# p2004dr/visual-slam

Measured on AMD Instinct MI355X. Metric: frames/sec (extract+match+pose) at 640×480, 2000 ORB, 1/2/4/8 MI355X, higher is better.
Workload: dtype u8

## Files before the change

### visual-slam_amd/csrc/orb_kernels.hip

```cpp
#include <type_traits>
#include <cstring>

#include "common.h"
#include "select_replay.h"
#include "fast_score.h"

__constant__ __attribute__((aligned(16))) int8_t c_pattern[256 * 4] = {
#include "orb_pattern.inc"
};

#define WAVE 64

__device__ __forceinline__ int reflect101(int p, int len) {
    if (len == 1) return 0;
    while (p < 0 || p >= len) p = p < 0 ? -p : 2 * len - 2 - p;
    return p;
}

__device__ __forceinline__ void xcd_map(uint32_t lin, uint32_t per, uint32_t inv_per, uint32_t batch, int& frame, int& item) {
    const uint32_t b8 = batch & ~7u, cut = per * b8;
    const bool head = lin < cut;
    const uint32_t n = head ? lin >> 3 : lin - cut;
    const uint32_t q = inv_per ? __umulhi(n, inv_per) : n;
    item = (int)(n - q * per);
// ... 915 lines not shown
                                              int* flags, replay::WgScratch<NT>* ws, uint32_t (*s_hw)[27] , int level) {
    const int tid = threadIdx.x;
    constexpr int HG_GROUPS = NT / HG;
    if ((lv.pitch & 3) == 0 && (((size_t)img) & 3) == 0) {
        const int grp = tid / HG, g = tid % HG;
#ifndef SEL_HB
#define SEL_HB 4
#endif
        constexpr int HB = SEL_HB;
        for (int i0 = 0; i0 < N1; i0 += HG_GROUPS * HB) {
            uint32_t e[HB], reg[HB][4];
#pragma unroll
            for (int u = 0; u < HB; u++) {
                e[u] = A[min(i0 + u * HG_GROUPS + grp, N1 - 1)];
                harris_fetch(img, lv.pitch, e[u] & 0xFFF, (e[u] >> 12) & 0xFFF, g, reg[u]);
            }
#pragma unroll
            for (int u = 0; u < HB; u++) {
                const int i = i0 + u * HG_GROUPS + grp;
                const float r = harris_group(reg[u], e[u] & 0xFFF, s_hw[grp], g);
                if (g == 0 && i < N1) B[i] = ((uint64_t)__float_as_uint(r) << 32) | (e[u] & 0xFFFFFFu);
            }
        }
    } else {
        for (int i = tid; i < N1; i += NT) {
            uint32_t e = A[i];
            int x = e & 0xFFF, y = (e >> 12) & 0xFFF;
            float r = harris_response(img, lv.pitch, x, y);
            B[i] = ((uint64_t)__float_as_uint(r) << 32) | (e & 0xFFFFFFu);
        }
    }
    __syncthreads();
    int N2 = replay::wg_retain_best<NT, uint64_t>(B, N1, lv.quota, P.select_order, rpos, bl, tid, ws);
    if (N2 > lv.fin_cap) {
        if (tid == 0) { atomicOr(&flags[0], 1); atomicOr(&flags[1], 1 << level); }
        N2 = lv.fin_cap;
    }
    for (int i = tid; i < N2; i += NT) {
        uint64_t e = B[i];
        FinalKp k;
        k.x = (uint16_t)(e & 0xFFF);
        k.y = (uint16_t)((e >> 12) & 0xFFF);
        k.response = __uint_as_float((uint32_t)(e >> 32));
        fin[i] = k;
    }
    if (tid == 0) *fin_cnt_out = N2;
}

template <int NT>
__global__ __launch_bounds__(NT) void k_select(Plan P, const uint8_t* __restrict__ gray, const uint8_t* __restrict__ pyr,
                                                        const uint32_t* __restrict__ cand, const int* __restrict__ strip_cnt,
                                                        uint64_t* __restrict__ scratch, size_t scratch_stride,
                                                        FinalKp* __restrict__ fin_all, int* __restrict__ fin_cnt, int* flags,
                                                        int level0, int buf_bytes, int* __restrict__ desc_todo) {
    extern __shared__ __attribute__((aligned(16))) uint8_t s_buf[];
    int* const s_pref = (int*)(s_buf + buf_bytes);
    __shared__ replay::WgScratch<NT> s_ws;
    __shared__ uint32_t s_hw[NT / HG][27];
    const int L = level0 + blockIdx.y, frame = blockIdx.x, tid = threadIdx.x;
    if (desc_todo && frame == 0 && blockIdx.y == 0 && tid == 0) desc_todo[0] = 0;
    const LevelInfo lv = P.lv[L];
    int* fin_cnt_out = &fin_cnt[(size_t)frame * MO_MAX_LEVELS + L];
    if (lv.nstrips == 0) {
        if (tid == 0) *fin_cnt_out = 0;
        return;
    }
    const int* cnts = strip_cnt + (size_t)frame * P.strips_per_frame + lv.strip_base;
    for (int s = tid; s < lv.nstrips; s += NT) s_pref[s + 1] = cnts[s];
    __syncthreads();
    if (tid == 0) {
        s_pref[0] = 0;
        for (int s = 0; s < lv.nstrips; s++) s_pref[s + 1] += s_pref[s];
    }
    __syncthreads();
    const int N = s_pref[lv.nstrips];
    uint64_t* scr = scratch + (size_t)frame * scratch_stride + lv.scr_off;
    uint64_t* gB = scr;
    uint32_t* gA = (uint32_t*)(scr + lv.cand_cap);
    uint16_t* g_rpos = (uint16_t*)(gA + lv.cand_cap + (lv.cand_cap & 1));
    unsigned long long* g_bl = (unsigned long long*)(g_rpos + (((size_t)lv.cand_cap / 2 + 4) & ~(size_t)3));
    const bool a_lds = sel_need_bytes(N, 4) <= (size_t)buf_bytes;
    uint32_t* s_A = (uint32_t*)s_buf;
    uint16_t* a_rpos = (uint16_t*)(s_buf + (((size_t)N * 4 + 7) & ~(size_t)7));
    unsigned long long* a_bl = (unsigned long long*)((uint8_t*)a_rpos + ((((size_t)N / 2 + 1) * 2 + 7) & ~(size_t)7));
    const uint32_t* src = cand + (size_t)frame * P.cand_stride + lv.cand_off;
    {
        const int lane = tid & 63, wv = tid >> 6;
        constexpr int NW = NT / 64, GU = 4;
        for (int s0 = wv; s0 < lv.nstrips; s0 += NW * GU) {
            uint32_t v[GU];
            int b[GU], n[GU];
#pragma unroll
            for (int u = 0; u < GU; u++) {
                const int st = min(s0 + u * NW, lv.nstrips - 1);
                b[u] = s_pref[st];
                n[u] = s0 + u * NW < lv.nstrips ? s_pref[st + 1] - b[u] : 0;
                v[u] = lane < n[u] ? src[(size_t)st * lv.strip_cap + lane] : 0u;
            }
#pragma unroll
            for (int u = 0; u < GU; u++) {
                if (lane < n[u]) { if (a_lds) s_A[b[u] + lane] = v[u]; else gA[b[u] + lane] = v[u]; }
                if (n[u] > WAVE) {
                    const uint32_t* e = src + (size_t)(s0 + u * NW) * lv.strip_cap;
                    for (int i = WAVE + lane; i < n[u]; i += WAVE) { if (a_lds) s_A[b[u] + i] = e[i]; else gA[b[u] + i] = e[i]; }
                }
            }
        }
    }
    __syncthreads();
    const int N1 = a_lds ? replay::wg_retain_best<NT, uint32_t>(s_A, N, 2 * lv.quota, P.select_order, a_rpos, a_bl, tid, &s_ws)
                         : replay::wg_retain_best<NT, uint32_t>(gA, N, 2 * lv.quota, P.select_order, g_rpos, g_bl, tid, &s_ws);
    const size_t b_off = a_lds ? (((size_t)N1 * 4 + 15) & ~(size_t)15) : 0;
    const bool b_lds = b_off + sel_need_bytes(N1, 8) <= (size_t)buf_bytes;
    uint64_t* s_B = (uint64_t*)(s_buf + b_off);
    uint16_t* b_rpos = (uint16_t*)((uint8_t*)s_B + (size_t)N1 * 8);
    unsigned long long* b_bl = (unsigned long long*)((uint8_t*)b_rpos + ((((size_t)N1 / 2 + 1) * 2 + 7) & ~(size_t)7));
    const uint8_t* img = level_ptr(P, L, gray, pyr, frame);
    FinalKp* fin = fin_all + (size_t)frame * P.fin_stride + lv.fin_off;
    if (a_lds && b_lds) select_harris<NT>(P, lv, img, s_A, s_B, N1, b_rpos, b_bl, fin, fin_cnt_out, flags, &s_ws, s_hw, L);
    else if (a_lds) select_harris<NT>(P, lv, img, s_A, gB, N1, g_rpos, g_bl, fin, fin_cnt_out, flags, &s_ws, s_hw, L);
    else if (b_lds) select_harris<NT>(P, lv, img, gA, s_B, N1, b_rpos, b_bl, fin, fin_cnt_out, flags, &s_ws, s_hw, L);
    else select_harris<NT>(P, lv, img, gA, gB, N1, g_rpos, g_bl, fin, fin_cnt_out, flags, &s_ws, s_hw, L);
}

int orb_launch_select(mo_ctx* c, const uint8_t* d_gray, int batch, int level_lo, int level_hi) {
    const Plan& P = c->plan;
    level_lo = std::max(level_lo, 0); level_hi = std::min(level_hi, P.nlevels);
    if (level_lo >= level_hi) return MO_OK;
    const size_t pref_bytes = (((size_t)c->pb.max_strips + 1) * sizeof(int) + 15) & ~(size_t)15;
    const size_t attr_bytes = SEL_BUF_BYTES + ((((size_t)SEL_MAXSTRIPS + 1) * sizeof(int) + 15) & ~(size_t)15);
    int rc;
    if ((rc = mo_raise_dyn_lds(c, (const void*)k_select<SEL_THREADS>, (int)attr_bytes)) ||
        (rc = mo_raise_dyn_lds(c, (const void*)k_select<SEL_THREADS_LATENCY>, (int)attr_bytes)))
        return rc;
    const dim3 grid(batch, level_hi - level_lo);
    if (batch <= 2)
        hipLaunchKernelGGL(k_select<SEL_THREADS_LATENCY>, grid, dim3(SEL_THREADS_LATENCY), SEL_BUF_BYTES + pref_bytes, c->stream, P, d_gray, c->pb.d_pyr, c->pb.d_cand,
                           c->pb.d_strip_cnt, c->pb.d_scratch, c->pb.scratch_stride, c->pb.d_fin, c->pb.d_fin_cnt, c->flags_cur, level_lo, SEL_BUF_BYTES, c->pb.d_dtodo);
    else
        hipLaunchKernelGGL(k_select<SEL_THREADS>, grid, dim3(SEL_THREADS), SEL_BUF_BYTES + pref_bytes, c->stream, P, d_gray, c->pb.d_pyr, c->pb.d_cand,
                           c->pb.d_strip_cnt, c->pb.d_scratch, c->pb.scratch_stride, c->pb.d_fin, c->pb.d_fin_cnt, c->flags_cur, level_lo, SEL_BUF_BYTES, c->pb.d_dtodo);
    HIPCHK(c, hipGetLastError());
    return MO_OK;
}

__global__ __launch_bounds__(SEL_THREADS) void k_retain_probe(const float* resp, int n, int n_points, int order, uint64_t* rec,
                                                              uint16_t* rpos, unsigned long long* bl, int32_t* out, int* nout) {
    __shared__ replay::WgScratch<SEL_THREADS> s_ws;
    for (int i = threadIdx.x; i < n; i += SEL_THREADS) rec[i] = ((uint64_t)__float_as_uint(resp[i]) << 32) | (uint32_t)i;
    __syncthreads();
    int keep = replay::wg_retain_best<SEL_THREADS, uint64_t>(rec, n, n_points, order, rpos, bl, threadIdx.x, &s_ws);
    __syncthreads();
    for (int i = threadIdx.x; i < keep; i += SEL_THREADS) out[i] = (int32_t)(rec[i] & 0xFFFFFFFFu);
    if (threadIdx.x == 0) *nout = keep;
}

int orb_launch_retain_probe(mo_ctx* c, const float* d_resp, int n, int n_points, int order, int32_t* d_order, int* d_nout) {
    size_t nn = (size_t)std::max(n, 1);
    size_t rec_b = nn * sizeof(uint64_t), rpos_b = ((nn / 2 + 4) * 2 + 7) & ~(size_t)7, bl_b = (nn / 64 + 8) * 8;
    int rc = c->d_tmp.reserve_exact(c, rec_b + rpos_b + bl_b);
    if (rc) return rc;
    uint8_t* b = c->d_tmp;
    hipLaunchKernelGGL(k_retain_probe, dim3(1), dim3(SEL_THREADS), 0, c->stream, d_resp, n, n_points, order, (uint64_t*)b,
                       (uint16_t*)(b + rec_b), (unsigned long long*)(b + rec_b + rpos_b), d_order, d_nout);
    HIPCHK(c, hipGetLastError());
    return MO_OK;
}

__device__ __forceinline__ float fast_atan2_deg(float y, float x) {
    const float p1 = 0.9997878412794807f * (float)(180 / 3.14159265358979323846);
    const float p3 = -0.3258083974640975f * (float)(180 / 3.14159265358979323846);
    const float p5 = 0.1555786518463281f * (float)(180 / 3.14159265358979323846);
    const float p7 = -0.04432655554792128f * (float)(180 / 3.14159265358979323846);
    float ax = fabsf(x), ay = fabsf(y);
    float a, c, c2;
    if (ax >= ay) {
        c = ay / (ax + (float)2.2204460492503131e-16);
        c2 = c * c;
        a = (((p7 * c2 + p5) * c2 + p3) * c2 + p1) * c;
    } else {
        c = ax / (ay + (float)2.2204460492503131e-16);
        c2 = c * c;
        a = 90.f - (((p7 * c2 + p5) * c2 + p3) * c2 + p1) * c;
    }
    if (x < 0) a = 180.f - a;
    if (y < 0) a = 360.f - a;
    return a;
}

__device__ __forceinline__ int wave_sum(int v) {
#pragma unroll
    for (int o = 32; o > 0; o >>= 1) v += __shfl_xor(v, o, 64);
    return v;
}

template <bool BOUNDS>
__device__ __forceinline__ void rbrief_wave(const uint8_t* blur, int bpitch, const uint8_t* raw, int rpitch, int lw, int lh,
                                            int cx, int cy, float angle_deg, uint8_t* desc, int lane) {
    float angle = angle_deg;
    angle *= (float)(3.14159265358979323846 / 180.f);
    double sd, cd;
    sincos((double)angle, &sd, &cd);
    float a = (float)cd, b = (float)sd;
    unsigned nib = 0;
#pragma unroll
    for (int k = 0; k < 4; k++) {
        const int8_t* pt = &c_pattern[(lane * 4 + k) * 4];
        float fx0 = (float)pt[0], fy0 = (float)pt[1], fx1 = (float)pt[2], fy1 = (float)pt[3];
        int ix0 = __float2int_rn(fx0 * a - fy0 * b), iy0 = __float2int_rn(fx0 * b + fy0 * a);
        int ix1 = __float2int_rn(fx1 * a - fy1 * b), iy1 = __float2int_rn(fx1 * b + fy1 * a);
        int x0 = cx + ix0, y0 = cy + iy0, x1 = cx + ix1, y1 = cy + iy1;
        int t0, t1;
        if (BOUNDS) {
            t0 = (x0 >= 0 && x0 < lw && y0 >= 0 && y0 < lh) ? blur[(size_t)y0 * bpitch + x0]
                                                           : raw[(size_t)reflect101(y0, lh) * rpitch + reflect101(x0, lw)];
            t1 = (x1 >= 0 && x1 < lw && y1 >= 0 && y1 < lh) ? blur[(size_t)y1 * bpitch + x1]
                                                           : raw[(size_t)reflect101(y1, lh) * rpitch + reflect101(x1, lw)];
        } else {
            t0 = blur[(size_t)y0 * bpitch + x0];
            t1 = blur[(size_t)y1 * bpitch + x1];
        }
        nib |= (t0 < t1 ? 1u : 0u) << k;
    }
    unsigned hi = __shfl_down(nib, 1, 64);
    if ((lane & 1) == 0) desc[lane >> 1] = (uint8_t)(nib | (hi << 4));
}

#define DG 16

__device__ __forceinline__ int group_sum(int v) {
#pragma unroll
    for (int o = DG / 2; o > 0; o >>= 1) v += __shfl_xor(v, o, 64);
    return v;
}

typedef const __attribute__((address_space(3))) uint8_t lds_cu8;
__device__ __forceinline__ uint16_t rbrief_u16_lds(uint32_t lds_base, int ppitch, float a, float b, const float4* pat, int gl) {
    const uint32_t base = lds_base - 0x4B400000u - 0x400000u * (uint32_t)ppitch;
    uint32_t val = 0;
#ifndef RB_UNROLL
#define RB_UNROLL 16
#endif
#pragma unroll 1
    for (int k0 = 16 - RB_UNROLL; k0 >= 0; k0 -= RB_UNROLL) {
#pragma unroll
        for (int kk = RB_UNROLL - 1; kk >= 0; kk--) {
            const float4 pt = pat[(k0 + kk) * DG + gl];
            const int jx0 = __float_as_int((pt.x * a - pt.y * b) + 12582912.f), jy0 = __float_as_int((pt.x * b + pt.y * a) + 12582912.f);
            const int jx1 = __float_as_int((pt.z * a - pt.w * b) + 12582912.f), jy1 = __float_as_int((pt.z * b + pt.w * a) + 12582912.f);
            const uint32_t a0 = (uint32_t)__mul24(jy0, ppitch) + (base + (uint32_t)jx0), a1 = (uint32_t)__mul24(jy1, ppitch) + (base + (uint32_t)jx1);
            const int t0 = *(lds_cu8*)(uintptr_t)a0, t1 = *(lds_cu8*)(uintptr_t)a1;
            val = __builtin_amdgcn_alignbit(val, (uint32_t)(t0 - t1), 31);
        }
    }
    return (uint16_t)val;
}

#define DT_RAW_P ((DT_W + 30 + 15 + 15) & ~15)
#define DT_RAW_ROWS (DT_H + 30)
#define DT_BLR_P ((DT_W + 38 + 15 + 15) & ~15)
#define DT_BLR_ROWS (DT_H + 38)
#define DT_RAW_NQ ((DT_W + 30 + 7 + 7) >> 3)
#define DT_BLR_NQ ((DT_W + 38 + 7 + 7) >> 3)
static_assert(((DT_RAW_P / 4) & 1) || ((DT_RAW_P / 4) & 7) == 4, "raw tile pitch: odd, or an odd multiple of 4 dwords");
#ifndef DT_NT
#define DT_NT 256
#endif
#ifdef DT_WAVES
#define DT_WAVES_ATTR __attribute__((amdgpu_waves_per_eu(DT_WAVES, 8)))
#else
#define DT_WAVES_ATTR
#endif
#define DT_CHUNK 512
#define DT_LIST (DT_NT > 160 ? DT_NT : 160)
#define DT_RAW_LD ((DT_RAW_ROWS * DT_RAW_NQ + DT_NT - 1) / DT_NT)
#define DT_BLR_LD ((DT_BLR_ROWS * DT_BLR_NQ + DT_NT - 1) / DT_NT)
#define DT_RAW_NP (DT_RAW_P / 16)
#define DT_BLR_NP (DT_BLR_P / 16)
#define DT_RAW_LD16 ((DT_RAW_ROWS + DT_NT / DT_RAW_NP - 1) / (DT_NT / DT_RAW_NP))
#define DT_BLR_LD16 ((DT_BLR_ROWS + DT_NT / DT_BLR_NP - 1) / (DT_NT / DT_BLR_NP))
#define DT_MAX2(a, b) ((a) > (b) ? (a) : (b))
#define DT_STAGE_REGS DT_MAX2(DT_MAX2(2 * DT_RAW_LD, 2 * DT_BLR_LD), DT_MAX2(4 * DT_RAW_LD16, 4 * DT_BLR_LD16))

template <int NROWS, int NQ, int NLD>
__device__ __forceinline__ void tile_issue(const uint8_t* img, int pitch, int h, int ry0, int cx_al, int tid, uint32_t (&v)[DT_STAGE_REGS]) {
    const int last_q = (pitch >> 3) - 1;
#pragma unroll
    for (int u = 0; u < NLD; u++) {
        const int t = min(tid + u * DT_NT, NROWS * NQ - 1), r = t / NQ, c = t - r * NQ;
        const int y = min(max(ry0 + r, 0), h - 1), q = min(max((cx_al >> 3) + c, 0), last_q);
        const uint2 d = ((const uint2*)(img + (size_t)y * pitch))[q];
        v[2 * u] = d.x; v[2 * u + 1] = d.y;
    }
}
template <int NROWS, int NQ, int LP, int NLD>
__device__ __forceinline__ void tile_store(uint8_t* lds, int tid, const uint32_t (&v)[DT_STAGE_REGS]) {
#pragma unroll
    for (int u = 0; u < NLD; u++) {
        const int t = tid + u * DT_NT, r = t / NQ, c = t - r * NQ;
        if (t < NROWS * NQ) *(uint2*)(lds + r * LP + 8 * c) = make_uint2(v[2 * u], v[2 * u + 1]);
    }
}
typedef uint32_t dt_u32x4 __attribute__((ext_vector_type(4)));
template <int NP>
__device__ __forceinline__ void tile_lane16(int pitch, int ry0, int cx_al, int nrows, int ncols, int tid, uint32_t& goff, uint32_t& loff, int& rows_left,
                                            uint32_t& last) {
    const int g = tid / NP, l = tid - g * NP;
    const bool on = g < DT_NT / NP && 16 * l < ncols && g < nrows;
    rows_left = on ? nrows - g : 0;
    goff = (uint32_t)(ry0 * pitch + cx_al) + (on ? (uint32_t)(g * pitch + 16 * l) : 0u);
    loff = (uint32_t)(g * (NP * 16) + 16 * l);
    last = on ? (uint32_t)((rows_left - 1) / (DT_NT / NP) * (DT_NT / NP) * pitch) : 0u;
}
template <int NP, int NLD>
__device__ __forceinline__ void tile_issue16(const uint8_t* img, int pitch, uint32_t goff, uint32_t last, uint32_t (&v)[DT_STAGE_REGS]) {
#pragma unroll
    for (int u = 0; u < NLD; u++) {
        const dt_u32x4 d = *(const dt_u32x4*)(img + (goff + min((uint32_t)(u * (DT_NT / NP) * pitch), last)));
        v[4 * u] = d.x; v[4 * u + 1] = d.y; v[4 * u + 2] = d.z; v[4 * u + 3] = d.w;
    }
}
template <int NP, int NLD>
__device__ __forceinline__ void tile_store16(uint8_t* lds, uint32_t loff, int rows_left, const uint32_t (&v)[DT_STAGE_REGS]) {
#pragma unroll
    for (int u = 0; u < NLD; u++)
        if (u * (DT_NT / NP) < rows_left) *(dt_u32x4*)(lds + loff + u * (DT_NT / NP) * (NP * 16)) = dt_u32x4{v[4 * u], v[4 * u + 1], v[4 * u + 2], v[4 * u + 3]};
}
__device__ __forceinline__ void tile_load_bytes(const uint8_t* img, int pitch, int w, int h, int ry0, int nrows, int cx0, int lp, uint8_t* lds, int tid) {
    for (int i = tid; i < nrows * lp; i += DT_NT) {
        const int r = i / lp, c = i - r * lp;
        const int y = min(max(ry0 + r, 0), h - 1), x = min(max(cx0 + c, 0), w - 1);
        lds[i] = img[(size_t)y * pitch + x];
    }
}

template <bool HAS_DESC, bool RARE>
__device__ __forceinline__ void describe_tile(const Plan& P, int frame, int tile, int tiles_per_frame, int split, int nsplit ,
                                              const uint32_t* __restrict__ tile_tab,
                                              const uint8_t* __restrict__ gray, const uint8_t* __restrict__ pyr,
                                              const uint8_t* __restrict__ blur, const FinalKp* __restrict__ fin_all,
                                              const int* __restrict__ fin_cnt, mo_keypoint* __restrict__ kps,
                                              uint8_t* __restrict__ desc, int cap, int* __restrict__ counts, int* flags,
                                              const uint32_t* __restrict__ icw, int* __restrict__ todo) {
    __shared__ __attribute__((aligned(16))) uint8_t s_tile[HAS_DESC ? DT_BLR_ROWS * DT_BLR_P : DT_RAW_ROWS * DT_RAW_P];
    __shared__ __attribute__((aligned(16))) float4 s_pat[HAS_DESC ? 256 : 1];
    __shared__ uint32_t s_list[DT_LIST];
    __shared__ float2 s_ab[DT_LIST];
    __shared__ int s_n;
    static_assert(DT_BLR_ROWS * DT_BLR_P >= DT_RAW_ROWS * DT_RAW_P, "the blurred tile is the larger one");
    const uint32_t te = tile_tab[tile];
    const int L = te & 0xFF;
    const int x0 = P.lv[L].bx0 + (int)((te >> 8) & 0xFFF) * DT_W, y0 = P.lv[L].by0 + (int)(te >> 20) * DT_H;
    const int lpitch = P.lv[L].pitch, lbpitch = P.lv[L].bpitch, lw = P.lv[L].w, lh = P.lv[L].h;
    const float lscale = P.lv[L].scale;
    const int tid = threadIdx.x, grp = tid / DG, gl = tid % DG;
    const int* fc = fin_cnt + (size_t)frame * MO_MAX_LEVELS;
    int total = 0, base = 0, nL = 0;
    {
        int cn[MO_MAX_LEVELS];
#pragma unroll
        for (int l = 0; l < MO_MAX_LEVELS; l++) cn[l] = fc[l];
#pragma unroll
        for (int l = 0; l < MO_MAX_LEVELS; l++) {
            const int n = l < P.nlevels ? cn[l] : 0;
            if (l == L) { base = total; nL = n; }
            total += n;
        }
    }
    if (!RARE && tile == 0 && split == 0 && tid == 0) {
        counts[frame] = total;
        if (total > cap) atomicOr(&flags[0], 2);
    }
    nL = min(nL, max(cap - base, 0));
    if (nL == 0) return;
    const uint8_t* img = level_ptr(P, L, gray, pyr, frame);
    const uint8_t* bl = blur + (size_t)frame * P.blur_stride + P.lv[L].boff;
    const bool al_raw = (lpitch & 7) == 0 && (((size_t)img) & 7) == 0;
    const bool al_blr = (((size_t)bl) & 7) == 0;
    const int nkc = min(DT_W, P.lv[L].bx0 + P.lv[L].bw - x0), nkr = min(DT_H, P.lv[L].by0 + P.lv[L].bh - y0);
    const int lead_r16 = (x0 - 15) & 15, lead_b16 = (x0 - 19) & 15;
    const int ncols_r = lead_r16 + nkc + 30, ncols_b = lead_b16 + nkc + 38;
    const bool w16_raw = !RARE && ((lpitch | (int)(size_t)img) & 15) == 0 && y0 - 15 >= 0 && y0 + nkr + 15 <= lh && x0 - 15 - lead_r16 >= 0 &&
                         x0 - 15 - lead_r16 + ((ncols_r + 15) & ~15) <= lpitch;
    const bool w16_blr = !RARE && ((lbpitch | (int)(size_t)bl) & 15) == 0 && y0 - 19 >= 0 && y0 + nkr + 19 <= lh && x0 - 19 - lead_b16 >= 0 &&
                         x0 - 19 - lead_b16 + ((ncols_b + 15) & ~15) <= lbpitch;
    const int xr_al = w16_raw ? x0 - 15 - lead_r16 : al_raw ? (x0 - 15) & ~7 : x0 - 15, lead_r = (x0 - 15) - xr_al;
    const int xb_al = w16_blr ? x0 - 19 - lead_b16 : al_blr ? (x0 - 19) & ~7 : x0 - 19;
    const FinalKp* fin = fin_all + (size_t)frame * P.fin_stride + P.lv[L].fin_off;
    FinalKp fk[DT_CHUNK / DT_NT];
    uint32_t vs[DT_STAGE_REGS];
    uint32_t goff = 0, loff = 0, last = 0;
    int rows_left = 0;
    if (!RARE) {
#pragma unroll
        for (int u = 0; u < DT_CHUNK / DT_NT; u++) fk[u] = fin[min(tid + u * DT_NT, nL - 1)];
        if (w16_raw) {
            tile_lane16<DT_RAW_NP>(lpitch, y0 - 15, xr_al, nkr + 30, ncols_r, tid, goff, loff, rows_left, last);
            tile_issue16<DT_RAW_NP, DT_RAW_LD16>(img, lpitch, goff, last, vs);
        } else if (al_raw) tile_issue<DT_RAW_ROWS, DT_RAW_NQ, DT_RAW_LD>(img, lpitch, lh, y0 - 15, xr_al, tid, vs);
    }
    uint32_t wt[8], mk[8];
    auto load_icw = [&]() {
        const uint4* w = (const uint4*)(icw + gl * 16);
        const uint4 w0 = w[0], w1 = w[1], k0 = w[2], k1 = w[3];
        wt[0] = w0.x; wt[1] = w0.y; wt[2] = w0.z; wt[3] = w0.w; wt[4] = w1.x; wt[5] = w1.y; wt[6] = w1.z; wt[7] = w1.w;
        mk[0] = k0.x; mk[1] = k0.y; mk[2] = k0.z; mk[3] = k0.w; mk[4] = k1.x; mk[5] = k1.y; mk[6] = k1.z; mk[7] = k1.w;
    };
    if (HAS_DESC && tid < 256 && DT_NT >= 256) {
        const int l = tid & 15, k = tid >> 4;
        const int8_t* pt = &c_pattern[(l * 16 + k) * 4];
        s_pat[k * DG + l] = make_float4((float)pt[0], (float)pt[1], (float)pt[2], (float)pt[3]);
    } else if (HAS_DESC && DT_NT < 256) {
        for (int i = tid; i < 256; i += DT_NT) {
            const int l = i & 15, k = i >> 4;
            const int8_t* pt = &c_pattern[(l * 16 + k) * 4];
            s_pat[k * DG + l] = make_float4((float)pt[0], (float)pt[1], (float)pt[2], (float)pt[3]);
        }
    }
    const int row_b_w = gl == 15 ? 0 : 1;
    const uint32_t tile_lds = (uint32_t)(uintptr_t)s_tile;

    auto select = [&](int c0, int sub) {
#pragma unroll
        for (int u = 0; u < DT_CHUNK / DT_NT; u++) {
            const int i = c0 + tid + u * DT_NT;
            const int dx = (int)fk[u].x - x0, dy = (int)fk[u].y - y0;
            if ((sub < 0 || u == sub) && i < nL && (unsigned)dx < DT_W && (unsigned)dy < DT_H && (i & (nsplit - 1)) == split) {
                const int pos = atomicAdd(&s_n, 1);
                if (pos < DT_LIST) {
                    s_list[pos] = (uint32_t)(i - c0) | ((uint32_t)dx << 9) | ((uint32_t)dy << 17);
                    s_ab[pos].y = fk[u].response;
                }
            }
        }
    };
    auto phase_a = [&](int c0, int n) {
        for (int j = grp; j < n; j += DT_NT / DG) {
            const uint32_t e = s_list[j];
            const int i = c0 + (int)(e & 0x1FF), dx = (int)((e >> 9) & 255), dy = (int)(e >> 17);
            const int k = base + i, x = x0 + dx, y = y0 + dy;
            const int col = dx + lead_r, offr = col & 3;
            int m10 = 0, m01 = 0;
#pragma unroll
            for (int rr = 0; rr < 2; rr++) {
                const int row_i = rr == 0 ? gl : 30 - gl;
                const uint32_t* rowp = (const uint32_t*)(s_tile + (dy + row_i) * DT_RAW_P + (col & ~3));
                uint32_t pxw[9];
#pragma unroll
                for (int c4 = 0; c4 < 9; c4++) pxw[c4] = rowp[c4];
                uint32_t sw = 0, rs = 0;
#pragma unroll
                for (int c4 = 0; c4 < 8; c4++) {
                    const uint32_t a = __builtin_amdgcn_alignbyte(pxw[c4 + 1], pxw[c4], (uint32_t)offr);
                    sw = __builtin_amdgcn_udot4(a, wt[c4], sw, false);
                    rs = __builtin_amdgcn_udot4(a, mk[c4], rs, false);
                }
                const int wgt = rr == 0 ? 1 : row_b_w;
                m10 += wgt * ((int)sw - 16 * (int)rs);
                m01 += wgt * (row_i - 15) * (int)rs;
            }
            m10 = group_sum(m10);
            m01 = group_sum(m01);
            const float angle = fast_atan2_deg((float)m01, (float)m10);
            if (gl == 0) {
                mo_keypoint* o = kps + (size_t)frame * cap + k;
                o->x = (float)x * lscale; o->y = (float)y * lscale;
                o->size = 31 * lscale;
                o->angle = angle;
                o->response = s_ab[j].y;
                o->octave = L;
                o->class_id = -1;
                s_ab[j].x = angle;
            }
        }
    };
    auto phase_b = [&](int n) {
        for (int j = tid; j < n; j += DT_NT) {
            float angle = s_ab[j].x;
            angle *= (float)(3.14159265358979323846 / 180.f);
            double sd, cd;
            sincos((double)angle, &sd, &cd);
            s_ab[j] = make_float2((float)cd, (float)sd);
        }
    };
    auto phase_c = [&](int c0, int n) {
        for (int j = grp; j < n; j += DT_NT / DG) {
            const uint32_t ex = s_list[j];
            const int i = c0 + (int)(ex & 0x1FF), dx = (int)((ex >> 9) & 255), dy = (int)(ex >> 17);
            const int k = base + i;
            const float px = (float)(x0 + dx) * lscale, py = (float)(y0 + dy) * lscale, inv = 1.f / lscale;
            const int cx = __float2int_rn(px * inv), cy = __float2int_rn(py * inv);
            const float2 ab = s_ab[j];
            int glo = gl;
            asm volatile("" : "+v"(glo));
            *(uint16_t*)(desc + ((size_t)frame * cap + k) * 32 + 2 * gl) =
                rbrief_u16_lds(tile_lds + (uint32_t)((cy - (y0 - 19)) * DT_BLR_P + (cx - xb_al)), DT_BLR_P, ab.x, ab.y, s_pat, glo);
        }
    };

    if (!RARE) {
        if (tid == 0) s_n = 0;
        if (w16_raw) tile_store16<DT_RAW_NP, DT_RAW_LD16>(s_tile, loff, rows_left, vs);
        else if (al_raw) tile_store<DT_RAW_ROWS, DT_RAW_NQ, DT_RAW_P, DT_RAW_LD>(s_tile, tid, vs);
        else tile_load_bytes(img, lpitch, lw, lh, y0 - 15, DT_RAW_ROWS, xr_al, DT_RAW_P, s_tile, tid);
        load_icw();
        __syncthreads();
        select(0, -1);
        __syncthreads();
        const int n0 = s_n;
        if (nL > DT_CHUNK || n0 > DT_LIST) {
            if (tid == 0 && (split == 0 || n0 > DT_LIST)) todo[1 + atomicAdd(&todo[0], 1)] = frame * tiles_per_frame + tile;
            return;
        }
        phase_a(0, n0);
        if (HAS_DESC) {
            if (w16_blr) {
                tile_lane16<DT_BLR_NP>(lbpitch, y0 - 19, xb_al, nkr + 38, ncols_b, tid, goff, loff, rows_left, last);
                tile_issue16<DT_BLR_NP, DT_BLR_LD16>(bl, lbpitch, goff, last, vs);
            } else if (al_blr) tile_issue<DT_BLR_ROWS, DT_BLR_NQ, DT_BLR_LD>(bl, lbpitch, lh, y0 - 19, xb_al, tid, vs);
            __syncthreads();
            phase_b(n0);
            if (w16_blr) tile_store16<DT_BLR_NP, DT_BLR_LD16>(s_tile, loff, rows_left, vs);
            else if (al_blr) tile_store<DT_BLR_ROWS, DT_BLR_NQ, DT_BLR_P, DT_BLR_LD>(s_tile, tid, vs);
            else tile_load_bytes(bl, lbpitch, lw, lh, y0 - 19, DT_BLR_ROWS, xb_al, DT_BLR_P, s_tile, tid);
            __syncthreads();
            phase_c(0, n0);
        }
        return;
    }
    load_icw();
    for (int c0 = 0; c0 < nL; c0 += DT_CHUNK) {
#pragma unroll
        for (int u = 0; u < DT_CHUNK / DT_NT; u++) fk[u] = fin[min(c0 + tid + u * DT_NT, nL - 1)];
#pragma unroll 1
        for (int sub = 0; sub < DT_CHUNK / DT_NT; sub++) {
            __syncthreads();
            if (tid == 0) s_n = 0;
            tile_load_bytes(img, lpitch, lw, lh, y0 - 15, DT_RAW_ROWS, xr_al, DT_RAW_P, s_tile, tid);
            __syncthreads();
            select(c0, sub);
            __syncthreads();
            const int n = s_n;
            phase_a(c0, n);
            if (HAS_DESC) {
                __syncthreads();
                tile_load_bytes(bl, lbpitch, lw, lh, y0 - 19, DT_BLR_ROWS, xb_al, DT_BLR_P, s_tile, tid);
                phase_b(n);
                __syncthreads();
                phase_c(c0, n);
            }
        }
    }
    __syncthreads();
}

template <bool HAS_DESC>
__global__ __launch_bounds__(DT_NT) DT_WAVES_ATTR void k_describe_tiles(Plan P, const uint32_t* __restrict__ tile_tab, uint32_t inv_per,
                                                          const uint8_t* __restrict__ gray, const uint8_t* __restrict__ pyr,
                                                          const uint8_t* __restrict__ blur, const FinalKp* __restrict__ fin_all,
                                                          const int* __restrict__ fin_cnt, mo_keypoint* __restrict__ kps,
                                                          uint8_t* __restrict__ desc, int cap, int* __restrict__ counts, int* flags,
                                                          const uint32_t* __restrict__ icw, int* __restrict__ todo) {
    int frame = blockIdx.y, tile = blockIdx.x;
    xcd_map(blockIdx.x + gridDim.x * blockIdx.y, gridDim.x, inv_per, gridDim.y, frame, tile);
    describe_tile<HAS_DESC, false>(P, frame, tile, (int)gridDim.x, (int)blockIdx.z, (int)gridDim.z, tile_tab, gray, pyr, blur, fin_all, fin_cnt, kps, desc, cap, counts, flags, icw, todo);
}

template <bool HAS_DESC>
__global__ __launch_bounds__(DT_NT) void k_describe_tiles_rare(Plan P, const uint32_t* __restrict__ tile_tab, int tiles_per_frame,
                                                               const uint8_t* __restrict__ gray, const uint8_t* __restrict__ pyr,
                                                               const uint8_t* __restrict__ blur, const FinalKp* __restrict__ fin_all,
                                                               const int* __restrict__ fin_cnt, mo_keypoint* __restrict__ kps,
                                                               uint8_t* __restrict__ desc, int cap, int* __restrict__ counts, int* flags,
                                                               const uint32_t* __restrict__ icw, int* __restrict__ todo) {
    const int n = todo[0];
    for (int e = blockIdx.x; e < n; e += gridDim.x) {
        const int ft = todo[1 + e];
        describe_tile<HAS_DESC, true>(P, ft / tiles_per_frame, ft % tiles_per_frame, tiles_per_frame, 0, 1, tile_tab, gray, pyr, blur, fin_all, fin_cnt, kps,
                                      desc, cap, counts, flags, icw, todo);
    }
}

int orb_launch_describe(mo_ctx* c, const uint8_t* d_gray, int batch, mo_keypoint* d_kps, uint8_t* d_desc, int cap, int* d_counts) {
    const Plan& P = c->plan;
    if (c->pb.n_dtiles == 0) {
        HIPCHK(c, hipMemsetAsync(d_counts, 0, (size_t)batch * sizeof(int), c->stream));
        return MO_OK;
    }
    const dim3 grid(c->pb.n_dtiles, batch, batch <= 2 ? DT_SPLIT_LATENCY : 1);
    const uint32_t inv_per = grid.x > 1 ? 0xFFFFFFFFu / grid.x + 1u : 0u;
    const uint32_t* const dtile_tab = c->pb.d_tables + c->pb.dtile_tab;
    const uint32_t* icw = c->pb.d_tables + c->pb.dtile_icw;
    const dim3 rare_grid(std::min(c->pb.n_dtiles * batch, 256));
    if (d_desc) {
        hipLaunchKernelGGL(k_describe_tiles<true>, grid, dim3(DT_NT), 0, c->stream, P, dtile_tab, inv_per, d_gray, c->pb.d_pyr, c->pb.d_blur,
                           c->pb.d_fin, c->pb.d_fin_cnt, d_kps, d_desc, cap, d_counts, c->flags_cur, icw, c->pb.d_dtodo);
        hipLaunchKernelGGL(k_describe_tiles_rare<true>, rare_grid, dim3(DT_NT), 0, c->stream, P, dtile_tab, c->pb.n_dtiles, d_gray, c->pb.d_pyr,
                           c->pb.d_blur, c->pb.d_fin, c->pb.d_fin_cnt, d_kps, d_desc, cap, d_counts, c->flags_cur, icw, c->pb.d_dtodo);
    } else {
        hipLaunchKernelGGL(k_describe_tiles<false>, grid, dim3(DT_NT), 0, c->stream, P, dtile_tab, inv_per, d_gray, c->pb.d_pyr, c->pb.d_blur,
                           c->pb.d_fin, c->pb.d_fin_cnt, d_kps, d_desc, cap, d_counts, c->flags_cur, icw, c->pb.d_dtodo);
        hipLaunchKernelGGL(k_describe_tiles_rare<false>, rare_grid, dim3(DT_NT), 0, c->stream, P, dtile_tab, c->pb.n_dtiles, d_gray, c->pb.d_pyr,
                           c->pb.d_blur, c->pb.d_fin, c->pb.d_fin_cnt, d_kps, d_desc, cap, d_counts, c->flags_cur, icw, c->pb.d_dtodo);
    }
    HIPCHK(c, hipGetLastError());
    return MO_OK;
}

#define DC_TILE_BYTES 13312
#define DC_MAXREC 256
__global__ __launch_bounds__(256) void k_describe_cells(Plan P, const uint8_t* __restrict__ blur, const mo_keypoint* __restrict__ kps,
                                                        const int32_t* __restrict__ kbase, uint8_t* __restrict__ desc, int cap, int cw,
                                                        int ch, int tpitch) {
    __shared__ __attribute__((aligned(16))) uint8_t s_tile[DC_TILE_BYTES];
    __shared__ __attribute__((aligned(16))) float4 s_pat[256];
    __shared__ float2 s_ab[DC_MAXREC];
    __shared__ uint32_t s_ctr[DC_MAXREC];
    const int cell = blockIdx.x, frame = blockIdx.y, tid = threadIdx.x, grp = tid / DG, gl = tid % DG;
    const int i0 = kbase[(size_t)frame * 65 + cell], n = min(kbase[(size_t)frame * 65 + cell + 1] - i0, DC_MAXREC);
    if (n <= 0) return;
    const int x0 = (cell & 7) * cw, y0 = (cell >> 3) * ch;
    const LevelInfo lv = P.lv[0];
    const uint8_t* bl = blur + (size_t)frame * P.blur_stride + lv.boff;
    const int xb_al = (x0 - 19) & ~7, rows = ch + 38, nq = tpitch >> 3, last_q = (lv.bpitch >> 3) - 1;
    {
        constexpr int U = 8;
        const int total = rows * nq;
        const uint32_t inv = 0xFFFFFFFFu / (uint32_t)nq + 1u;
        for (int t0 = tid; t0 < total; t0 += 256 * U) {
            uint2 v[U];
#pragma unroll
            for (int u = 0; u < U; u++) {
                const int t = min(t0 + u * 256, total - 1), r = (int)__umulhi((uint32_t)t, inv), c = t - r * nq;
                const int y = min(max(y0 - 19 + r, 0), lv.h - 1), q = min(max((xb_al >> 3) + c, 0), last_q);
                v[u] = ((const uint2*)(bl + (size_t)y * lv.bpitch))[q];
            }
#pragma unroll
            for (int u = 0; u < U; u++) {
                const int t = t0 + u * 256, r = (int)__umulhi((uint32_t)t, inv), c = t - r * nq;
                if (t < total) *(uint2*)(s_tile + r * tpitch + 8 * c) = v[u];
            }
        }
    }
    {
        const int l = tid & 15, k = tid >> 4;
        const int8_t* pt = &c_pattern[(l * 16 + k) * 4];
        s_pat[k * DG + l] = make_float4((float)pt[0], (float)pt[1], (float)pt[2], (float)pt[3]);
    }
    const uint32_t tile_lds = (uint32_t)(uintptr_t)s_tile;
    for (int j = tid; j < n; j += 256) {
        const mo_keypoint kp = kps[(size_t)frame * cap + i0 + j];
        const float inv = 1.f / lv.scale;
        const int cx = __float2int_rn(kp.x * inv), cy = __float2int_rn(kp.y * inv);
        float angle = kp.angle;
        angle *= (float)(3.14159265358979323846 / 180.f);
        double sd, cd;
        sincos((double)angle, &sd, &cd);
        s_ab[j] = make_float2((float)cd, (float)sd);
        s_ctr[j] = tile_lds + (uint32_t)((cy - (y0 - 19)) * tpitch + (cx - xb_al));
    }
    __syncthreads();
    for (int j = grp; j < n; j += 256 / DG) {
        const float2 ab = s_ab[j];
        int glo = gl;
        asm volatile("" : "+v"(glo));
        *(uint16_t*)(desc + ((size_t)frame * cap + i0 + j) * 32 + 2 * gl) = rbrief_u16_lds(s_ctr[j], tpitch, ab.x, ab.y, s_pat, glo);
    }
}

int orb_launch_describe_cells(mo_ctx* c, const mo_keypoint* d_kps, const int32_t* d_kbase, uint8_t* d_desc, int cap, int batch) {
    const Plan& P = c->plan;
    const int cw = P.w / 8, ch = P.h / 8;
    const int tpitch = (cw + 38 + 7 + 7) & ~7;
    if ((size_t)tpitch * (ch + 38) > DC_TILE_BYTES || P.edge_threshold < 19) return MO_ERR_UNSUPPORTED;
    hipLaunchKernelGGL(k_describe_cells, dim3(64, batch), dim3(256), 0, c->stream, P, c->pb.d_blur, d_kps, d_kbase, d_desc, cap, cw, ch, tpitch);
    HIPCHK(c, hipGetLastError());
    return MO_OK;
}

__global__ __launch_bounds__(256) void k_describe_given(Plan P, const uint8_t* __restrict__ gray,
                                                        const uint8_t* __restrict__ pyr, const uint8_t* __restrict__ blur,
                                                        const mo_keypoint* __restrict__ kps, int n, const int* __restrict__ n_dev,
                                                        int n_stride, uint8_t* __restrict__ desc) {
    const int lane = threadIdx.x & 63, frame = blockIdx.y;
    const int k = blockIdx.x * 4 + (threadIdx.x >> 6);
    const int cap = n;
    if (n_dev) n = min(n, n_dev[(size_t)frame * n_stride]);
    if (k >= n) return;
    mo_keypoint kp = kps[(size_t)frame * cap + k];
    const int L = kp.octave;
    const LevelInfo lv = P.lv[L];
    float inv = 1.f / lv.scale;
    int cx = __float2int_rn(kp.x * inv), cy = __float2int_rn(kp.y * inv);
    const uint8_t* img = level_ptr(P, L, gray, pyr, frame);
    const uint8_t* bl = blur + (size_t)frame * P.blur_stride + lv.boff;
    rbrief_wave<true>(bl, lv.bpitch, img, lv.pitch, lv.w, lv.h, cx, cy, kp.angle, desc + ((size_t)frame * cap + k) * 32, lane);
}

int orb_launch_describe_given(mo_ctx* c, const uint8_t* d_gray, const mo_keypoint* d_kps, int n, uint8_t* d_desc, const int* d_n, int batch,
                              int n_stride) {
    if (n <= 0) return MO_OK;
    const Plan& P = c->plan;
    hipLaunchKernelGGL(k_describe_given, dim3((n + 3) / 4, batch), dim3(256), 0, c->stream, P, d_gray, c->pb.d_pyr, c->pb.d_blur, d_kps,
                       n, d_n, n_stride, d_desc);
    HIPCHK(c, hipGetLastError());
    return MO_OK;
}
```

Baseline: 126,400.

## Compute BRIEF descriptor with one wavefront per keypoint using ballot bits

Phase C now gives each keypoint a whole 64-lane wavefront. Each lane evaluates four of the 256 pattern comparisons, keeping the pattern points in registers loaded from constant memory, and `__ballot` packs the results into the 32-byte descriptor. A single lane writes it with two 16-byte stores. The LDS pattern table and its setup go away. The atan2 orientation moves out of the group-wide phase A into per-keypoint phase B, which also precomputes the sample base offset with float-magic rounding tricks. The costs are more scalar readfirstlane traffic and a dependence on exact bit tricks for the rounding and offsets.

```diff
diff --git a/visual-slam_amd/csrc/orb_kernels.hip b/visual-slam_amd/csrc/orb_kernels.hip
--- a/visual-slam_amd/csrc/orb_kernels.hip
+++ b/visual-slam_amd/csrc/orb_kernels.hip
@@ -1241,6 +1241,7 @@
     }
 }
 typedef uint32_t dt_u32x4 __attribute__((ext_vector_type(4)));
+typedef dt_u32x4 dt_u32x4_a4 __attribute__((aligned(4)));
 template <int NP>
 __device__ __forceinline__ void tile_lane16(int pitch, int ry0, int cx_al, int nrows, int ncols, int tid, uint32_t& goff, uint32_t& loff, int& rows_left,
                                             uint32_t& last) {
@@ -1282,7 +1283,6 @@
                                               uint8_t* __restrict__ desc, int cap, int* __restrict__ counts, int* flags,
                                               const uint32_t* __restrict__ icw, int* __restrict__ todo) {
     __shared__ __attribute__((aligned(16))) uint8_t s_tile[HAS_DESC ? DT_BLR_ROWS * DT_BLR_P : DT_RAW_ROWS * DT_RAW_P];
-    __shared__ __attribute__((aligned(16))) float4 s_pat[HAS_DESC ? 256 : 1];
     __shared__ uint32_t s_list[DT_LIST];
     __shared__ float2 s_ab[DT_LIST];
     __shared__ int s_n;
@@ -1345,17 +1345,11 @@
         wt[0] = w0.x; wt[1] = w0.y; wt[2] = w0.z; wt[3] = w0.w; wt[4] = w1.x; wt[5] = w1.y; wt[6] = w1.z; wt[7] = w1.w;
         mk[0] = k0.x; mk[1] = k0.y; mk[2] = k0.z; mk[3] = k0.w; mk[4] = k1.x; mk[5] = k1.y; mk[6] = k1.z; mk[7] = k1.w;
     };
-    if (HAS_DESC && tid < 256 && DT_NT >= 256) {
-        const int l = tid & 15, k = tid >> 4;
-        const int8_t* pt = &c_pattern[(l * 16 + k) * 4];
-        s_pat[k * DG + l] = make_float4((float)pt[0], (float)pt[1], (float)pt[2], (float)pt[3]);
-    } else if (HAS_DESC && DT_NT < 256) {
-        for (int i = tid; i < 256; i += DT_NT) {
-            const int l = i & 15, k = i >> 4;
-            const int8_t* pt = &c_pattern[(l * 16 + k) * 4];
-            s_pat[k * DG + l] = make_float4((float)pt[0], (float)pt[1], (float)pt[2], (float)pt[3]);
-        }
-    }
+    uint32_t pq[4] = {0, 0, 0, 0};
+    auto load_pat = [&]() {
+#pragma unroll
+        for (int r = 0; r < 4; r++) pq[r] = ((const uint32_t*)c_pattern)[64 * r + (tid & 63)];
+    };
     const int row_b_w = gl == 15 ? 0 : 1;
     const uint32_t tile_lds = (uint32_t)(uintptr_t)s_tile;
 
@@ -1400,40 +1394,67 @@
             }
             m10 = group_sum(m10);
             m01 = group_sum(m01);
-            const float angle = fast_atan2_deg((float)m01, (float)m10);
+            const float angle = HAS_DESC ? 0.f : fast_atan2_deg((float)m01, (float)m10);
             if (gl == 0) {
                 mo_keypoint* o = kps + (size_t)frame * cap + k;
                 o->x = (float)x * lscale; o->y = (float)y * lscale;
                 o->size = 31 * lscale;
-                o->angle = angle;
+                if (!HAS_DESC) o->angle = angle;
                 o->response = s_ab[j].y;
                 o->octave = L;
                 o->class_id = -1;
-                s_ab[j].x = angle;
+                if (HAS_DESC) s_ab[j] = make_float2(__int_as_float(m01), __int_as_float(m10));
             }
         }
     };
-    auto phase_b = [&](int n) {
+    auto phase_b = [&](int c0, int n) {
         for (int j = tid; j < n; j += DT_NT) {
-            float angle = s_ab[j].x;
+            const float2 mm = s_ab[j];
+            float angle = fast_atan2_deg((float)__float_as_int(mm.x), (float)__float_as_int(mm.y));
+            kps[(size_t)frame * cap + base + c0 + (int)(s_list[j] & 0x1FF)].angle = angle;
             angle *= (float)(3.14159265358979323846 / 180.f);
             double sd, cd;
             sincos((double)angle, &sd, &cd);
             s_ab[j] = make_float2((float)cd, (float)sd);
-        }
-    };
-    auto phase_c = [&](int c0, int n) {
-        for (int j = grp; j < n; j += DT_NT / DG) {
             const uint32_t ex = s_list[j];
-            const int i = c0 + (int)(ex & 0x1FF), dx = (int)((ex >> 9) & 255), dy = (int)(ex >> 17);
-            const int k = base + i;
+            const int dx = (int)((ex >> 9) & 255), dy = (int)(ex >> 17);
             const float px = (float)(x0 + dx) * lscale, py = (float)(y0 + dy) * lscale, inv = 1.f / lscale;
             const int cx = __float2int_rn(px * inv), cy = __float2int_rn(py * inv);
-            const float2 ab = s_ab[j];
-            int glo = gl;
-            asm volatile("" : "+v"(glo));
-            *(uint16_t*)(desc + ((size_t)frame * cap + k) * 32 + 2 * gl) =
-                rbrief_u16_lds(tile_lds + (uint32_t)((cy - (y0 - 19)) * DT_BLR_P + (cx - xb_al)), DT_BLR_P, ab.x, ab.y, s_pat, glo);
+            s_list[j] = (ex & 0x1FF) | ((uint32_t)((cy - (y0 - 19)) * DT_BLR_P + (cx - xb_al)) << 9);
+        }
+    };
+    auto phase_c = [&](int c0, int nv) {
+        static_assert(DT_NT % 64 == 0, "phase C works in whole wavefronts");
+        static_assert(DT_BLR_ROWS * DT_BLR_P < (1 << 23), "sample offset beside the 9-bit index");
+        const int n = __builtin_amdgcn_readfirstlane(nv), wv = __builtin_amdgcn_readfirstlane(tid >> 6);
+        float4 pt[4];
+#pragma unroll
+        for (int r = 0; r < 4; r++) {
+            asm volatile("" : "+v"(pq[r]));
+            pt[r] = make_float4((float)(int8_t)pq[r], (float)(int8_t)(pq[r] >> 8), (float)(int8_t)(pq[r] >> 16), (float)(int8_t)(pq[r] >> 24));
+        }
+        for (int j = wv; j < n; j += DT_NT / 64) {
+            const uint32_t ex = (uint32_t)__builtin_amdgcn_readfirstlane((int)s_list[j]);
+            const float2 abv = s_ab[j];
+            const float a = __int_as_float(__builtin_amdgcn_readfirstlane(__float_as_int(abv.x)));
+            const float b = __int_as_float(__builtin_amdgcn_readfirstlane(__float_as_int(abv.y)));
+            const int k = base + c0 + (int)(ex & 0x1FF);
+            const uint32_t sb = tile_lds + (ex >> 9) - 0x4B400000u - 0x400000u * (uint32_t)DT_BLR_P;
+            uint32_t m[8];
+#pragma unroll
+            for (int r = 0; r < 4; r++) {
+                const int jx0 = __float_as_int((pt[r].x * a - pt[r].y * b) + 12582912.f), jy0 = __float_as_int((pt[r].x * b + pt[r].y * a) + 12582912.f);
+                const int jx1 = __float_as_int((pt[r].z * a - pt[r].w * b) + 12582912.f), jy1 = __float_as_int((pt[r].z * b + pt[r].w * a) + 12582912.f);
+                const uint32_t a0 = (uint32_t)__mul24(jy0, DT_BLR_P) + (sb + (uint32_t)jx0), a1 = (uint32_t)__mul24(jy1, DT_BLR_P) + (sb + (uint32_t)jx1);
+                const int t0 = *(lds_cu8*)(uintptr_t)a0, t1 = *(lds_cu8*)(uintptr_t)a1;
+                const unsigned long long bits = __ballot(t0 < t1);
+                m[2 * r] = (uint32_t)bits; m[2 * r + 1] = (uint32_t)(bits >> 32);
+            }
+            if ((tid & 63) == 0) {
+                dt_u32x4_a4* o = (dt_u32x4_a4*)(desc + ((size_t)frame * cap + k) * 32);
+                o[0] = dt_u32x4{m[0], m[1], m[2], m[3]};
+                o[1] = dt_u32x4{m[4], m[5], m[6], m[7]};
+            }
         }
     };
 
@@ -1457,8 +1478,9 @@
                 tile_lane16<DT_BLR_NP>(lbpitch, y0 - 19, xb_al, nkr + 38, ncols_b, tid, goff, loff, rows_left, last);
                 tile_issue16<DT_BLR_NP, DT_BLR_LD16>(bl, lbpitch, goff, last, vs);
             } else if (al_blr) tile_issue<DT_BLR_ROWS, DT_BLR_NQ, DT_BLR_LD>(bl, lbpitch, lh, y0 - 19, xb_al, tid, vs);
+            load_pat();
             __syncthreads();
-            phase_b(n0);
+            phase_b(0, n0);
             if (w16_blr) tile_store16<DT_BLR_NP, DT_BLR_LD16>(s_tile, loff, rows_left, vs);
             else if (al_blr) tile_store<DT_BLR_ROWS, DT_BLR_NQ, DT_BLR_P, DT_BLR_LD>(s_tile, tid, vs);
             else tile_load_bytes(bl, lbpitch, lw, lh, y0 - 19, DT_BLR_ROWS, xb_al, DT_BLR_P, s_tile, tid);
@@ -1482,9 +1504,10 @@
             const int n = s_n;
             phase_a(c0, n);
             if (HAS_DESC) {
+                load_pat();
                 __syncthreads();
                 tile_load_bytes(bl, lbpitch, lw, lh, y0 - 19, DT_BLR_ROWS, xb_al, DT_BLR_P, s_tile, tid);
-                phase_b(n);
+                phase_b(c0, n);
                 __syncthreads();
                 phase_c(c0, n);
             }
```

Result: faster. 128,000 (median of 6 runs) (+1.2%).
